# jafarinia/snuffy

Measured on AMD Instinct MI355X. Metric: slides/sec, higher is better.
Workload: dtype f32; 1 GPU; cfgB: MILNet eval forward, 1 bag/step/rank, N=32768 patches D=768 h=6 Lambda=200 (K=200) depth=1 relu mlp x4; parallelism=bag-parallel x1, bags_resident_per_rank=8, launch=hip graph replay, rccl_ranks=0

## Files before the change

### snuffy_amd/csrc/rowops.hip

```cpp
#include <math.h>

#include "common.h"
#include "philox.h"
#include "selector.h"

namespace {

constexpr int WG = 256;
constexpr int WAVES = WG / 64;

template <int VEC>
struct VecT;
template <>
struct VecT<4> {
    using type = float4;
};
template <>
struct VecT<1> {
    using type = float;
};

template <int VEC, int NV>
struct RowRegs {
    float v[NV * VEC];
// ... 27 lines not shown
                *reinterpret_cast<float4*>(row + e) = make_float4(r[i * 4], r[i * 4 + 1], r[i * 4 + 2], r[i * 4 + 3]);
            } else {
                row[e] = r[i];
            }
        }
    }
}

template <int VEC, int NV>
__device__ __forceinline__ void store_row_bf16(unsigned short* __restrict__ row, int d, int lane,
                                               const float (&r)[NV * VEC]) {
#pragma unroll
    for (int i = 0; i < NV; ++i) {
        int e = (i * 64 + lane) * VEC;
        if (e < d) {
            if constexpr (VEC == 4) {
                uint2 p;
                p.x = pack_bf16x2(r[i * 4], r[i * 4 + 1]);
                p.y = pack_bf16x2(r[i * 4 + 2], r[i * 4 + 3]);
                *reinterpret_cast<uint2*>(row + e) = p;
            } else {
                row[e] = f32_to_bf16_bits(r[i]);
            }
        }
    }
}

template <int VEC, int NV, int LN>
__global__ __launch_bounds__(WG) void critic_kernel(const float* __restrict__ x, int64_t n, int d,
                                                    const float* __restrict__ w, const float* __restrict__ b,
                                                    int c_out, float* __restrict__ scores, float eps,
                                                    unsigned short* __restrict__ xhat,
                                                    unsigned int* __restrict__ sel_hist,
                                                    const float* __restrict__ gamma = nullptr,
                                                    const float* __restrict__ beta = nullptr) {
    const int lane = threadIdx.x & 63;
    const int wave = threadIdx.x >> 6;
    const float inv_d = 1.0f / (float)d;
    __shared__ unsigned int s_hist[snf::SEL_BINS];
    if (sel_hist) {
        for (int i = threadIdx.x; i < snf::SEL_BINS; i += WG) s_hist[i] = 0;
        __syncthreads();
    }
    float w0[NV * VEC];
    load_row<VEC, NV>(w, d, lane, w0);
    const float b0 = b ? b[0] : 0.f;
// ... 35 lines not shown
            for (int i = 0; i < NV; ++i) {
#pragma unroll
                for (int t = 0; t < VEC; ++t) {
                    int e = (i * 64 + lane) * VEC + t;
                    float dv = (e < d) ? (r[i * VEC + t] - mean) : 0.f;
                    s2 = fmaf(dv, dv, s2);
                }
            }
            const float var = wave_sum(s2) * inv_d;
            const float rstd = 1.0f / sqrtf(var + eps);
#pragma unroll
            for (int i = 0; i < NV * VEC; ++i) r[i] = (r[i] - mean) * rstd;
            if constexpr (LN == 1) store_row_bf16<VEC, NV>(xhat + row * d, d, lane, r);
            if constexpr (LN == 2 && VEC == 4) {
                if (gamma) {
                    float g[NV * VEC], bt[NV * VEC];
                    load_row<VEC, NV>(gamma, d, lane, g);
                    load_row<VEC, NV>(beta, d, lane, bt);
#pragma unroll
                    for (int i = 0; i < NV * VEC; ++i) {
                        r[i] = fmaf(r[i], g[i], bt[i]);
                    }
                }
                unsigned short* o2 = xhat + row * 2 * d;
#pragma unroll
                for (int i = 0; i < NV; ++i) {
                    const int e = (i * 64 + lane) * 4;
                    if (e < d) {
                        uint2 hi, lo;
                        hi.x = pack_bf16x2(r[i * 4], r[i * 4 + 1]);
                        hi.y = pack_bf16x2(r[i * 4 + 2], r[i * 4 + 3]);
                        lo.x = pack_bf16x2(r[i * 4] - __uint_as_float(hi.x << 16), r[i * 4 + 1] - __uint_as_float(hi.x & 0xffff0000u));
                        lo.y = pack_bf16x2(r[i * 4 + 2] - __uint_as_float(hi.y << 16), r[i * 4 + 3] - __uint_as_float(hi.y & 0xffff0000u));
                        unsigned short* o = o2 + 64 * (e >> 5) + (e & 31);
                        *reinterpret_cast<uint2*>(o) = hi;
                        *reinterpret_cast<uint2*>(o + 32) = lo;
                    }
                }
            }
        }
    }
    if (sel_hist) {
        __syncthreads();
        unsigned int* g = sel_hist + (blockIdx.x & (snf::SEL_REPL - 1)) * snf::SEL_BINS;
        for (int i = threadIdx.x; i < snf::SEL_BINS; i += WG) {
            const unsigned int c = s_hist[i];
            if (c) __hip_atomic_fetch_add(&g[i], c, __ATOMIC_RELAXED, __HIP_MEMORY_SCOPE_AGENT);
        }
    }
}

__global__ __launch_bounds__(1024) void colmax_kernel(const float* __restrict__ scores, int64_t n, int c_out,
                                                      float* __restrict__ out_val, int64_t* __restrict__ out_idx) {
    const int c = blockIdx.x;
    float best = -INFINITY;
    int64_t bi = INT64_MAX;
    bool has_nan = false;
    int64_t nan_i = INT64_MAX;
    for (int64_t i = threadIdx.x; i < n; i += blockDim.x) {
        float v = scores[i * c_out + c];
        if (v != v) {
// ... 81 lines not shown
        }
        const float var = wave_sum(s2) * inv_d;
        const float rstd = 1.0f / sqrtf(var + eps);
#pragma unroll
        for (int i = 0; i < NV * VEC; ++i) {
            float v = (r[i] - mean) * rstd;
            if (gamma) v *= g[i];
            if (beta) v += bt[i];
            r[i] = v;
        }
        const int64_t orow = out_row_idx ? out_row_idx[row] : row;
        if (out_f32) store_row_f32<VEC, NV>(out_f32 + orow * d, d, lane, r);
        if (out_bf16 && !split3) store_row_bf16<VEC, NV>(out_bf16 + orow * d, d, lane, r);
        if (out_bf16 && split3 == 1) {
            float lo[NV * VEC];
#pragma unroll
            for (int i = 0; i < NV * VEC; ++i) lo[i] = r[i] - bf16_bits_to_f32(f32_to_bf16_bits(r[i]));
            unsigned short* o3 = out_bf16 + orow * 3 * d;
            store_row_bf16<VEC, NV>(o3, d, lane, r);
            store_row_bf16<VEC, NV>(o3 + d, d, lane, r);
            store_row_bf16<VEC, NV>(o3 + 2 * d, d, lane, lo);
        }
        if constexpr (VEC == 4) {
            if (out_bf16 && split3 == 2) {
                unsigned short* o2 = out_bf16 + orow * 2 * d;
#pragma unroll
                for (int i = 0; i < NV; ++i) {
                    const int e = (i * 64 + lane) * 4;
                    if (e < d) {
                        uint2 hi, lo;
                        hi.x = pack_bf16x2(r[i * 4], r[i * 4 + 1]);
                        hi.y = pack_bf16x2(r[i * 4 + 2], r[i * 4 + 3]);
                        lo.x = pack_bf16x2(r[i * 4] - __uint_as_float(hi.x << 16), r[i * 4 + 1] - __uint_as_float(hi.x & 0xffff0000u));
                        lo.y = pack_bf16x2(r[i * 4 + 2] - __uint_as_float(hi.y << 16), r[i * 4 + 3] - __uint_as_float(hi.y & 0xffff0000u));
                        unsigned short* o = o2 + 64 * (e >> 5) + (e & 31);
                        *reinterpret_cast<uint2*>(o) = hi;
                        *reinterpret_cast<uint2*>(o + 32) = lo;
                    }
                }
            }
        }
        if (lane == 0) {
            if (mean_out) mean_out[orow] = mean;
            if (rstd_out) rstd_out[orow] = rstd;
        }
    }
}

template <int VEC, int NV>
__device__ __forceinline__ void load_row_bf16(const unsigned short* __restrict__ row, int d, int lane, float (&r)[NV * VEC]) {
#pragma unroll
    for (int i = 0; i < NV; ++i) {
        int e = (i * 64 + lane) * VEC;
        if constexpr (VEC == 4) {
            uint2 t = make_uint2(0u, 0u);
            if (e < d) t = *reinterpret_cast<const uint2*>(row + e);
            r[i * 4 + 0] = __uint_as_float(t.x << 16);
            r[i * 4 + 1] = __uint_as_float(t.x & 0xffff0000u);
            r[i * 4 + 2] = __uint_as_float(t.y << 16);
            r[i * 4 + 3] = __uint_as_float(t.y & 0xffff0000u);
        } else {
            r[i] = (e < d) ? bf16_bits_to_f32(row[e]) : 0.f;
        }
// ... 721 lines not shown
    for (int i = 0; i < NV; ++i) {
        int e = (i * 64 + lane) * VEC;
        if (e < d) {
            if constexpr (VEC == 4) {
                uint2 p = *reinterpret_cast<const uint2*>(row + e);
                r[i * 4 + 0] += __uint_as_float(p.x << 16);
                r[i * 4 + 1] += __uint_as_float(p.x & 0xffff0000u);
                r[i * 4 + 2] += __uint_as_float(p.y << 16);
                r[i * 4 + 3] += __uint_as_float(p.y & 0xffff0000u);
            } else {
                r[i] += bf16_bits_to_f32(row[e]);
            }
        }
    }
}

template <int VEC, int NV, bool DEFER = false>
__global__ __launch_bounds__(WG) void ln_colsum_kernel(const float* __restrict__ z, int64_t n, int d, float eps,
                                                       const unsigned short* __restrict__ add_bf16,
                                                       const float* __restrict__ add_bias,
                                                       const int32_t* __restrict__ slot_map,
                                                       const float* __restrict__ delta_rows,
                                                       float* __restrict__ z_out,
                                                       float* __restrict__ partial ,
                                                       const int* __restrict__ vl = nullptr, int vl_bags = 0,
                                                       const float* __restrict__ slabs = nullptr,
                                                       const int32_t* __restrict__ tile_map = nullptr, int tiles_n = 0) {
    const int lane = threadIdx.x & 63;
    const int wave = threadIdx.x >> 6;
    int bid = blockIdx.x, gdim = gridDim.x;
    if (vl) {
        const int* __restrict__ dsc = vl + 4 * vl[4 * vl_bags + bid];
        const int64_t row0 = dsc[1];
        bid -= dsc[0];
        n = dsc[2];
        gdim = dsc[3];
        z += row0 * d;
        if (add_bf16) add_bf16 += row0 * d;
        if (slot_map) slot_map += row0;
        if (z_out) z_out += row0 * d;
    }
    float acc[NV * VEC];
#pragma unroll
    for (int i = 0; i < NV * VEC; ++i) acc[i] = 0.f;
    float bias_r[NV * VEC];
    if (add_bias) load_row<VEC, NV>(add_bias, d, lane, bias_r);
    const float inv_d = 1.0f / (float)d;
    const int64_t rstride = (int64_t)gdim * WAVES;
    float nz[NV * VEC];
    uint2 nb[NV];
    constexpr int NCB = DEFER ? (NV * VEC * 64 + 255) / 256 : 1;
    float ns[DEFER ? NV * VEC : 1];
    int mp_n[NCB], mp_nn[NCB];
    auto lookup = [&](int64_t row, int (&mp)[NCB]) __attribute__((always_inline)) {
        const int trow = __builtin_amdgcn_readfirstlane((int)(row >> 8));
#pragma unroll
        for (int cb = 0; cb < NCB; ++cb) mp[cb] = cb < tiles_n ? tile_map[(int64_t)trow * tiles_n + cb] : 0;
    };
    auto issue = [&](int64_t row) __attribute__((always_inline)) {
        load_row<VEC, NV>(z + row * d, d, lane, nz);
        if constexpr (DEFER) {
#pragma unroll
            for (int i = 0; i < NV; ++i) {
                const int sl = mp_n[i * 64 * VEC / 256];
#pragma unroll
                for (int t = 0; t < VEC; ++t) ns[i * VEC + t] = 0.f;
                if (sl) {
                    const int e = (i * 64 + lane) * VEC;
                    const float* __restrict__ sp = slabs + ((int64_t)(sl - 1) * 256 + (row & 255)) * 256 + (e & 255);
                    if constexpr (VEC == 4) {
                        if (e < d) {
                            const float4 t4 = *reinterpret_cast<const float4*>(sp);
                            ns[i * 4 + 0] = t4.x, ns[i * 4 + 1] = t4.y, ns[i * 4 + 2] = t4.z, ns[i * 4 + 3] = t4.w;
                        }
                    } else {
                        if (e < d) ns[i] = *sp;
                    }
                }
            }
        }
        if constexpr (VEC == 4) {
            if (add_bf16) {
#pragma unroll
                for (int i = 0; i < NV; ++i) {
                    const int e = (i * 64 + lane) * 4;
                    nb[i] = (e < d) ? *reinterpret_cast<const uint2*>(add_bf16 + row * d + e) : make_uint2(0u, 0u);
                }
            }
        }
    };
    int64_t row = (int64_t)bid * WAVES + wave;
    if constexpr (DEFER) {
        if (row < n) lookup(row, mp_n);
    }
    if (row < n) issue(row);
    if constexpr (DEFER) {
        if (row + rstride < n) lookup(row + rstride, mp_nn);
    }
    for (; row < n; row += rstride) {
        float r[NV * VEC];
#pragma unroll
        for (int i = 0; i < NV * VEC; ++i) r[i] = nz[i];
        if constexpr (DEFER) {
#pragma unroll
            for (int i = 0; i < NV; ++i) {
                if (mp_n[i * 64 * VEC / 256]) {
#pragma unroll
                    for (int t = 0; t < VEC; ++t) r[i * VEC + t] += ns[i * VEC + t];
                }
            }
#pragma unroll
            for (int cb = 0; cb < NCB; ++cb) mp_n[cb] = mp_nn[cb];
        }
        if constexpr (VEC == 4) {
            if (add_bf16) {
#pragma unroll
                for (int i = 0; i < NV; ++i) {
                    r[i * 4 + 0] += __uint_as_float(nb[i].x << 16);
                    r[i * 4 + 1] += __uint_as_float(nb[i].x & 0xffff0000u);
                    r[i * 4 + 2] += __uint_as_float(nb[i].y << 16);
                    r[i * 4 + 3] += __uint_as_float(nb[i].y & 0xffff0000u);
                }
            }
        } else {
            if (add_bf16) add_row_bf16<VEC, NV>(add_bf16 + row * d, d, lane, r);
        }
        if (row + rstride < n) issue(row + rstride);
        if constexpr (DEFER) {
            if (row + 2 * rstride < n) lookup(row + 2 * rstride, mp_nn);
        }
        if (add_bias) {
#pragma unroll
            for (int i = 0; i < NV * VEC; ++i) r[i] += bias_r[i];
        }
        if (slot_map) {
            int sl = slot_map[row];
            if (sl >= 0) {
                float dr[NV * VEC];
                load_row<VEC, NV>(delta_rows + (int64_t)sl * d, d, lane, dr);
#pragma unroll
                for (int i = 0; i < NV * VEC; ++i) r[i] += dr[i];
            }
        }
        if (z_out) store_row_f32<VEC, NV>(z_out + row * d, d, lane, r);
        float s1 = 0.f;
#pragma unroll
        for (int i = 0; i < NV * VEC; ++i) s1 += r[i];
        const float mean = wave_sum(s1) * inv_d;
        float s2 = 0.f;
#pragma unroll
        for (int i = 0; i < NV; ++i) {
#pragma unroll
            for (int t = 0; t < VEC; ++t) {
                int e = (i * 64 + lane) * VEC + t;
                float dv = (e < d) ? (r[i * VEC + t] - mean) : 0.f;
                s2 = fmaf(dv, dv, s2);
            }
        }
        const float rstd = 1.0f / sqrtf(wave_sum(s2) * inv_d + eps);
#pragma unroll
        for (int i = 0; i < NV * VEC; ++i) acc[i] += (r[i] - mean) * rstd;
    }
    extern __shared__ float lds[];
    float* mine = lds + wave * (NV * VEC * 64);
#pragma unroll
    for (int i = 0; i < NV * VEC; ++i) mine[i * 64 + lane] = acc[i];
    __syncthreads();
    if (wave == 0) {
#pragma unroll
        for (int i = 0; i < NV; ++i) {
#pragma unroll
            for (int t = 0; t < VEC; ++t) {
                float s = 0.f;
                for (int w2 = 0; w2 < WAVES; ++w2) s += lds[w2 * (NV * VEC * 64) + (i * VEC + t) * 64 + lane];
                int e = (i * 64 + lane) * VEC + t;
                if (e < d) partial[(int64_t)blockIdx.x * d + e] = s;
            }
        }
    }
}

constexpr int HEAD_NSLICE = 16;
__global__ __launch_bounds__(256) void ln_colreduce_kernel(const float* __restrict__ partial, int nparts, int d,
                                                           float* __restrict__ partial2 ,
                                                           const int* __restrict__ vl = nullptr) {
    __shared__ float red[4][64];
    if (vl) {
        const int* __restrict__ dsc = vl + 4 * blockIdx.z;
        partial += (int64_t)dsc[0] * d;
        nparts = dsc[3];
        partial2 += (int64_t)blockIdx.z * HEAD_NSLICE * d;
    }
    const int c = threadIdx.x & 63, wv = threadIdx.x >> 6;
    const int e = blockIdx.x * 64 + c;
    const int sl = blockIdx.y;
    float s = 0.f;
    if (e < d)
        for (int p = sl + HEAD_NSLICE * wv; p < nparts; p += HEAD_NSLICE * 4) s += partial[(int64_t)p * d + e];
    red[wv][c] = s;
    __syncthreads();
    if (wv == 0 && e < d) partial2[(int64_t)sl * d + e] = ((red[0][c] + red[1][c]) + red[2][c]) + red[3][c];
// ... 42 lines not shown
        const int opts[] = {1, 2, 3, 4, 6, 8};
        for (int o : opts)
            if (o >= need) {
                *cfg = {4, o};
                return true;
            }
        return false;
    }
    int need = (d + 63) / 64;
    const int opts[] = {1, 2, 3, 4, 8, 16, 32};
    for (int o : opts)
        if (o >= need) {
            *cfg = {1, o};
            return true;
        }
    return false;
}

inline int row_grid(int64_t n) {
    int64_t want = (n + WAVES - 1) / WAVES;
    int64_t cap = (int64_t)snf::cu_count() * 8;
    return (int)(want < cap ? (want > 0 ? want : 1) : cap);
}

#define SNF_ROW_DISPATCH(cfg, ...)                                \
    do {                                                          \
        if (cfg.vec == 4) {                                       \
            switch (cfg.nv) {                                     \
                case 1: { constexpr int VEC = 4, NV = 1; __VA_ARGS__; } break; \
                case 2: { constexpr int VEC = 4, NV = 2; __VA_ARGS__; } break; \
                case 3: { constexpr int VEC = 4, NV = 3; __VA_ARGS__; } break; \
                case 4: { constexpr int VEC = 4, NV = 4; __VA_ARGS__; } break; \
                case 6: { constexpr int VEC = 4, NV = 6; __VA_ARGS__; } break; \
                default: { constexpr int VEC = 4, NV = 8; __VA_ARGS__; } break; \
            }                                                     \
        } else {                                                  \
            switch (cfg.nv) {                                     \
                case 1: { constexpr int VEC = 1, NV = 1; __VA_ARGS__; } break; \
                case 2: { constexpr int VEC = 1, NV = 2; __VA_ARGS__; } break; \
                case 3: { constexpr int VEC = 1, NV = 3; __VA_ARGS__; } break; \
                case 4: { constexpr int VEC = 1, NV = 4; __VA_ARGS__; } break; \
                case 8: { constexpr int VEC = 1, NV = 8; __VA_ARGS__; } break; \
                case 16: { constexpr int VEC = 1, NV = 16; __VA_ARGS__; } break; \
                default: { constexpr int VEC = 1, NV = 32; __VA_ARGS__; } break; \
            }                                                     \
        }                                                         \
// ... 84 lines not shown
}

__global__ __launch_bounds__(256) void mil_loss_bwd_kernel(const float* __restrict__ grad_out, const float* __restrict__ fwd, const int64_t* __restrict__ argmax,
                                                           int64_t n, int c, float* __restrict__ d_ins, float* __restrict__ small) {
    const float go = grad_out[0];
    const int64_t total = n * c;
    for (int64_t i = (int64_t)blockIdx.x * 256 + threadIdx.x; i < total; i += (int64_t)gridDim.x * 256) {
        const int64_t row = i / c;
        const int j = (int)(i - row * c);
        d_ins[i] = row == argmax[j] ? go * fwd[2 + 2 * c + j] : 0.f;
    }
    if (blockIdx.x == 0 && threadIdx.x <= c) small[threadIdx.x] = go * (threadIdx.x < c ? fwd[2 + c + threadIdx.x] : fwd[1]);
}

extern "C" {

int snf_critic_f32(const float* x, int64_t n, int d, const float* w, const float* b, int c_out, float* scores,
                   float* colmax_val, int64_t* colmax_idx, snf_stream_t stream) {
    SNF_REQUIRE(x && w && scores, "snf_critic_f32: null pointer");
    SNF_REQUIRE(n >= 1 && d >= 1 && c_out >= 1, "snf_critic_f32: bad shape n=%lld d=%d c=%d", (long long)n, d, c_out);
    RowCfg cfg;
    SNF_REQUIRE(pick_row_cfg(d, aligned16(x) && aligned16(w), &cfg), "snf_critic_f32: d=%d too wide (max 2048)", d);
    hipStream_t s = snf::as_stream(stream);
    SNF_ROW_DISPATCH(cfg, hipLaunchKernelGGL((critic_kernel<VEC, NV, 0>), dim3(row_grid(n)), dim3(WG), 0, s, x, n, d, w,
                                              b, c_out, scores, 0.f, (unsigned short*)nullptr, (unsigned int*)nullptr));
    int rc = snf::check_launch("critic_kernel");
    if (rc) return rc;
    if (colmax_val || colmax_idx) {
        hipLaunchKernelGGL(colmax_kernel, dim3(c_out), dim3(1024), 0, s, scores, n, c_out, colmax_val, colmax_idx);
        rc = snf::check_launch("colmax_kernel");
    }
    return rc;
}

int snf_critic_ln_f32(const float* x, int64_t n, int d, const float* w, const float* b, int c_out, float* scores,
                      float eps, void* xhat_bf16, snf_stream_t stream) {
    SNF_REQUIRE(x && w && scores && xhat_bf16, "snf_critic_ln_f32: null pointer");
    SNF_REQUIRE(n >= 1 && d >= 1 && c_out >= 1, "snf_critic_ln_f32: bad shape n=%lld d=%d c=%d", (long long)n, d, c_out);
    RowCfg cfg;
    SNF_REQUIRE(pick_row_cfg(d, aligned16(x) && aligned16(w) && aligned16(xhat_bf16), &cfg),
                "snf_critic_ln_f32: d=%d too wide (max 2048)", d);
    hipStream_t s = snf::as_stream(stream);
    SNF_ROW_DISPATCH(cfg, hipLaunchKernelGGL((critic_kernel<VEC, NV, 1>), dim3(row_grid(n)), dim3(WG), 0, s, x, n, d, w,
                                              b, c_out, scores, eps, reinterpret_cast<unsigned short*>(xhat_bf16),
                                              (unsigned int*)nullptr));
    return snf::check_launch("critic_kernel<ln>");
}

int snf_critic_select_f32(const float* x, int64_t n, int d, const float* w, const float* b, float* scores, float eps,
                          void* xhat_bf16, void* selector_state, snf_stream_t stream) {
    SNF_REQUIRE(x && w && scores && selector_state, "snf_critic_select_f32: null pointer");
    SNF_REQUIRE(n >= 1 && d >= 1, "snf_critic_select_f32: bad shape n=%lld d=%d", (long long)n, d);
    SNF_REQUIRE(aligned16(selector_state), "snf_critic_select_f32: state must be 16-byte aligned");
    RowCfg cfg;
    SNF_REQUIRE(pick_row_cfg(d, aligned16(x) && aligned16(w) && (!xhat_bf16 || aligned16(xhat_bf16)), &cfg),
                "snf_critic_select_f32: d=%d too wide (max 2048)", d);
    hipStream_t s = snf::as_stream(stream);
    unsigned int* hist = reinterpret_cast<snf::SelectorState*>(selector_state)->hist;
    if (xhat_bf16) {
        SNF_ROW_DISPATCH(cfg, hipLaunchKernelGGL((critic_kernel<VEC, NV, 1>), dim3(row_grid(n)), dim3(WG), 0, s, x, n, d, w, b,
                                                  1, scores, eps, reinterpret_cast<unsigned short*>(xhat_bf16), hist));
    } else {
        SNF_ROW_DISPATCH(cfg, hipLaunchKernelGGL((critic_kernel<VEC, NV, 0>), dim3(row_grid(n)), dim3(WG), 0, s, x, n, d, w,
                                                  b, 1, scores, 0.f, (unsigned short*)nullptr, hist));
    }
    return snf::check_launch("critic_kernel<select>");
}

int snf_critic_ln_hl_f32(const float* x, int64_t n, int d, const float* w, const float* b, int c_out, float* scores,
                         const float* gamma, const float* beta, float eps, void* out_hl, void* selector_state,
                         snf_stream_t stream) {
    SNF_REQUIRE(x && w && scores && out_hl && (!gamma == !beta), "snf_critic_ln_hl_f32: null pointer (gamma and beta: both or neither)");
    SNF_REQUIRE(n >= 1 && d >= 32 && d % 32 == 0 && c_out >= 1, "snf_critic_ln_hl_f32: bad shape n=%lld d=%d c=%d (d % 32 == 0)",
                (long long)n, d, c_out);
    SNF_REQUIRE(!selector_state || (c_out == 1 && aligned16(selector_state)), "snf_critic_ln_hl_f32: the selector needs one class "
                "and a 16-byte aligned state");
    SNF_REQUIRE(aligned16(x) && aligned16(w) && (!gamma || (aligned16(gamma) && aligned16(beta))) && aligned16(out_hl),
                "snf_critic_ln_hl_f32: buffers must be 16-byte aligned");
    RowCfg cfg;
    SNF_REQUIRE(pick_row_cfg(d, true, &cfg) && cfg.vec == 4, "snf_critic_ln_hl_f32: d=%d too wide (max 2048)", d);
    hipStream_t s = snf::as_stream(stream);
    unsigned int* hist = selector_state ? reinterpret_cast<snf::SelectorState*>(selector_state)->hist : nullptr;
    switch (cfg.nv) {
#define SNF_CRITIC_HL_CASE(N)                                                                                              \
    case N:                                                                                                                 \
        hipLaunchKernelGGL((critic_kernel<4, N, 2>), dim3(row_grid(n)), dim3(WG), 0, s, x, n, d, w, b, c_out, scores, eps,  \
                           reinterpret_cast<unsigned short*>(out_hl), hist, gamma, beta);                                   \
        break;
        SNF_CRITIC_HL_CASE(1)
        SNF_CRITIC_HL_CASE(2)
        SNF_CRITIC_HL_CASE(3)
        SNF_CRITIC_HL_CASE(4)
        SNF_CRITIC_HL_CASE(6)
        default:
            SNF_CRITIC_HL_CASE(8)
#undef SNF_CRITIC_HL_CASE
    }
    return snf::check_launch("critic_kernel<ln, hl>");
}

int snf_layernorm_rows_f32(const float* x, int64_t n, int d, const int32_t* slot_map, const float* patch_rows,
                           const float* gamma, const float* beta, float eps, float* out_f32, void* out_bf16,
                           float* mean, float* rstd, const int64_t* out_row_idx, snf_stream_t stream) {
    SNF_REQUIRE(x, "snf_layernorm_rows_f32: null x");
    SNF_REQUIRE(n >= 1 && d >= 1, "snf_layernorm_rows_f32: bad shape");
    SNF_REQUIRE(!slot_map || patch_rows, "snf_layernorm_rows_f32: slot_map without patch_rows");
    bool al = aligned16(x) && (!patch_rows || aligned16(patch_rows)) && (!gamma || aligned16(gamma)) &&
              (!beta || aligned16(beta)) && (!out_f32 || aligned16(out_f32)) && (!out_bf16 || aligned16(out_bf16));
    RowCfg cfg;
    SNF_REQUIRE(pick_row_cfg(d, al, &cfg), "snf_layernorm_rows_f32: d=%d too wide (max 2048)", d);
    hipStream_t s = snf::as_stream(stream);
    SNF_ROW_DISPATCH(cfg, hipLaunchKernelGGL((layernorm_rows_kernel<VEC, NV>), dim3(row_grid(n)), dim3(WG), 0, s, x, n, d,
                                              slot_map, patch_rows, gamma, beta, eps, out_f32,
                                              reinterpret_cast<unsigned short*>(out_bf16), mean, rstd, out_row_idx, 0));
    return snf::check_launch("layernorm_rows_kernel");
}

int snf_layernorm_rows_split3_f32(const float* x, int64_t n, int d, const int32_t* slot_map, const float* patch_rows,
                                  const float* gamma, const float* beta, float eps, void* out_bf16, snf_stream_t stream) {
    SNF_REQUIRE(x && out_bf16, "snf_layernorm_rows_split3_f32: null pointer");
    SNF_REQUIRE(n >= 1 && d >= 1, "snf_layernorm_rows_split3_f32: bad shape");
    SNF_REQUIRE(!slot_map || patch_rows, "snf_layernorm_rows_split3_f32: slot_map without patch_rows");
    bool al = aligned16(x) && (!patch_rows || aligned16(patch_rows)) && (!gamma || aligned16(gamma)) &&
              (!beta || aligned16(beta)) && aligned16(out_bf16);
    RowCfg cfg;
    SNF_REQUIRE(pick_row_cfg(d, al, &cfg), "snf_layernorm_rows_split3_f32: d=%d too wide (max 2048)", d);
    hipStream_t s = snf::as_stream(stream);
    SNF_ROW_DISPATCH(cfg, hipLaunchKernelGGL((layernorm_rows_kernel<VEC, NV>), dim3(row_grid(n)), dim3(WG), 0, s, x, n, d,
                                              slot_map, patch_rows, gamma, beta, eps, (float*)nullptr,
                                              reinterpret_cast<unsigned short*>(out_bf16), (float*)nullptr, (float*)nullptr,
                                              (const int64_t*)nullptr, 1));
    return snf::check_launch("layernorm_rows_kernel<split3>");
}

int snf_layernorm_bwd_blocks(int64_t n) { return row_grid(n); }

int snf_layernorm_rows_bwd_f32(const float* x, int64_t n, int d, const void* dy, int dy_dtype, int64_t dy_stride,
                               const float* gamma, float eps, const float* residual, float* dx, void* dx_bf16,
                               float* partials, snf_stream_t stream) {
    SNF_REQUIRE(x && dy, "snf_layernorm_rows_bwd_f32: null pointer");
    SNF_REQUIRE(n >= 1 && d >= 1, "snf_layernorm_rows_bwd_f32: bad shape");
    SNF_REQUIRE(dy_dtype == SNF_DT_F32 || dy_dtype == SNF_DT_BF16, "snf_layernorm_rows_bwd_f32: bad dy dtype %d", dy_dtype);
    SNF_REQUIRE(dy_stride == 0 || dy_stride >= d, "snf_layernorm_rows_bwd_f32: bad dy row pitch");
    bool al = aligned16(x) && aligned16(dy) && (!gamma || aligned16(gamma)) && (!residual || aligned16(residual)) &&
              (!dx || aligned16(dx)) && (!dx_bf16 || aligned16(dx_bf16)) && dy_stride % 4 == 0;
    RowCfg cfg;
    SNF_REQUIRE(pick_row_cfg(d, al, &cfg), "snf_layernorm_rows_bwd_f32: d=%d too wide (max 2048)", d);
    hipStream_t s = snf::as_stream(stream);
    SNF_ROW_DISPATCH(cfg, hipLaunchKernelGGL((ln_bwd_rows_kernel<VEC, NV>), dim3(row_grid(n)), dim3(WG), 0, s, x, n, d, dy,
                                              dy_dtype == SNF_DT_BF16 ? 1 : 0, dy_stride, gamma, eps, residual, dx,
                                              reinterpret_cast<unsigned short*>(dx_bf16), partials));
// ... 109 lines not shown
            default: SNF_COLSUM_DROP(true, 4); break;
        }
    } else {
        switch (nch) {
            case 1: SNF_COLSUM_DROP(false, 1); break;
            case 2: SNF_COLSUM_DROP(false, 2); break;
            default: SNF_COLSUM_DROP(false, 4); break;
        }
    }
#undef SNF_COLSUM_DROP
    return snf::check_launch("colsum_fused_dropout_kernel");
}

int snf_layernorm_rows_hl_f32(const float* x, int64_t n, int d, const int32_t* slot_map, const float* patch_rows,
                              const float* gamma, const float* beta, float eps, void* out_bf16, snf_stream_t stream) {
    SNF_REQUIRE(x && out_bf16, "snf_layernorm_rows_hl_f32: null pointer");
    SNF_REQUIRE(n >= 1 && d >= 32 && d % 32 == 0, "snf_layernorm_rows_hl_f32: d=%d must be a multiple of 32", d);
    SNF_REQUIRE(!slot_map || patch_rows, "snf_layernorm_rows_hl_f32: slot_map without patch_rows");
    SNF_REQUIRE(aligned16(x) && (!patch_rows || aligned16(patch_rows)) && (!gamma || aligned16(gamma)) && (!beta || aligned16(beta)) &&
                    aligned16(out_bf16), "snf_layernorm_rows_hl_f32: buffers must be 16-byte aligned");
    RowCfg cfg;
    SNF_REQUIRE(pick_row_cfg(d, true, &cfg) && cfg.vec == 4, "snf_layernorm_rows_hl_f32: d=%d too wide (max 2048)", d);
    hipStream_t s = snf::as_stream(stream);
    SNF_ROW_DISPATCH(cfg, hipLaunchKernelGGL((layernorm_rows_kernel<VEC, NV>), dim3(row_grid(n)), dim3(WG), 0, s, x, n, d,
                                              slot_map, patch_rows, gamma, beta, eps, (float*)nullptr,
                                              reinterpret_cast<unsigned short*>(out_bf16), (float*)nullptr, (float*)nullptr,
                                              (const int64_t*)nullptr, 2));
    return snf::check_launch("layernorm_rows_kernel<hl>");
}

int snf_layernorm_rows_hl_patch_f32(const float* x, const float* addend, int64_t n, int d, const int64_t* out_row_idx,
                                    const float* gamma, const float* beta, float eps, void* out_hl, snf_stream_t stream) {
    SNF_REQUIRE(x && out_hl && out_row_idx, "snf_layernorm_rows_hl_patch_f32: null pointer");
    SNF_REQUIRE(n >= 1 && d >= 32 && d % 32 == 0, "snf_layernorm_rows_hl_patch_f32: d=%d must be a multiple of 32", d);
    SNF_REQUIRE(aligned16(x) && (!addend || aligned16(addend)) && (!gamma || aligned16(gamma)) && (!beta || aligned16(beta)) &&
                    aligned16(out_hl), "snf_layernorm_rows_hl_patch_f32: buffers must be 16-byte aligned");
    RowCfg cfg;
    SNF_REQUIRE(pick_row_cfg(d, true, &cfg) && cfg.vec == 4, "snf_layernorm_rows_hl_patch_f32: d=%d too wide (max 2048)", d);
    hipStream_t s = snf::as_stream(stream);
    SNF_ROW_DISPATCH(cfg, hipLaunchKernelGGL((layernorm_rows_kernel<VEC, NV>), dim3(row_grid(n)), dim3(WG), 0, s, x, n, d,
                                              (const int32_t*)nullptr, (const float*)nullptr, gamma, beta, eps, (float*)nullptr,
                                              reinterpret_cast<unsigned short*>(out_hl), (float*)nullptr, (float*)nullptr,
                                              out_row_idx, 2, addend));
    return snf::check_launch("layernorm_rows_kernel<hl patch>");
}

int snf_split_hl_f32(const float* x, int64_t ldx, int64_t m, int k, void* out_bf16, snf_stream_t stream) {
    SNF_REQUIRE(x && out_bf16, "snf_split_hl_f32: null pointer");
    SNF_REQUIRE(m >= 1 && k >= 32 && k % 32 == 0 && ldx >= k && ldx % 4 == 0, "snf_split_hl_f32: bad shape m=%lld k=%d ldx=%lld",
                (long long)m, k, (long long)ldx);
    SNF_REQUIRE(aligned16(x) && aligned16(out_bf16), "snf_split_hl_f32: buffers must be 16-byte aligned");
    const int64_t total = m * (k >> 3);
    int64_t blocks = (total + 255) / 256;
    const int64_t cap = (int64_t)snf::cu_count() * 16;
    if (blocks > cap) blocks = cap;
    hipLaunchKernelGGL(split_hl_kernel, dim3((int)blocks), dim3(256), 0, snf::as_stream(stream), x, ldx, m, k,
                       reinterpret_cast<unsigned short*>(out_bf16));
    return snf::check_launch("split_hl_kernel");
}

int snf_split3_f32(const float* x, int64_t ldx, int64_t m, int k, void* out_bf16, snf_stream_t stream) {
    SNF_REQUIRE(x && out_bf16, "snf_split3_f32: null pointer");
    SNF_REQUIRE(m >= 1 && k >= 8 && k % 8 == 0 && ldx >= k && ldx % 4 == 0, "snf_split3_f32: bad shape m=%lld k=%d ldx=%lld",
// ... 226 lines not shown

static int ln_mean_head_impl(const float* z, int64_t n, int d, const float* slabs, const int32_t* tile_map, int tiles_n,
                             const void* add_bf16, const float* add_bias, const int32_t* slot_map, const float* delta_rows,
                             float* z_out, const float* gamma, const float* beta, float eps, const float* w_head,
                             const float* b_head, int c_out, float* logits, float* pooled, void* workspace, size_t workspace_bytes,
                             snf_stream_t stream) {
    SNF_REQUIRE(z && w_head && logits && workspace, "snf_ln_mean_head_f32: null pointer");
    SNF_REQUIRE(!slot_map || delta_rows, "snf_ln_mean_head_f32: slot_map without delta_rows");
    SNF_REQUIRE(n >= 1 && d >= 1 && c_out >= 1, "snf_ln_mean_head_f32: bad shape");
    const int parts = ln_head_parts(n);
    if (workspace_bytes < ((size_t)parts + HEAD_NSLICE) * d * sizeof(float)) {
        snf::set_error("snf_ln_mean_head_f32: workspace %zu < %zu", workspace_bytes,
                       ((size_t)parts + HEAD_NSLICE) * d * sizeof(float));
        return SNF_EWORKSPACE;
    }
    RowCfg cfg;
    const bool al = aligned16(z) && (!add_bf16 || aligned16(add_bf16)) && (!add_bias || aligned16(add_bias)) &&
                    (!delta_rows || aligned16(delta_rows)) && (!z_out || aligned16(z_out));
    SNF_REQUIRE(pick_row_cfg(d, al, &cfg), "snf_ln_mean_head_f32: d=%d too wide (max 2048)", d);
    hipStream_t s = snf::as_stream(stream);
    float* partial = reinterpret_cast<float*>(workspace);
    float* partial2 = partial + (size_t)parts * d;
    if (tile_map) {
        SNF_ROW_DISPATCH(cfg, hipLaunchKernelGGL((ln_colsum_kernel<VEC, NV, true>), dim3(parts), dim3(WG),
                                                  WAVES * NV * VEC * 64 * sizeof(float), s, z, n, d, eps,
                                                  reinterpret_cast<const unsigned short*>(add_bf16), add_bias, slot_map,
                                                  delta_rows, z_out, partial, nullptr, 0, slabs, tile_map, tiles_n));
    } else {
        SNF_ROW_DISPATCH(cfg, hipLaunchKernelGGL((ln_colsum_kernel<VEC, NV>), dim3(parts), dim3(WG),
                                                  WAVES * NV * VEC * 64 * sizeof(float), s, z, n, d, eps,
                                                  reinterpret_cast<const unsigned short*>(add_bf16), add_bias, slot_map,
                                                  delta_rows, z_out, partial));
    }
    int rc = snf::check_launch("ln_colsum_kernel");
    if (rc) return rc;
    hipLaunchKernelGGL(ln_colreduce_kernel, dim3((d + 63) / 64, HEAD_NSLICE), dim3(256), 0, s, partial, parts, d, partial2);
    rc = snf::check_launch("ln_colreduce_kernel");
    if (rc) return rc;
    hipLaunchKernelGGL(head_gemv_kernel, dim3(c_out), dim3(256), 0, s, partial2, n, d, gamma, beta, w_head, b_head, pooled,
                       logits);
    return snf::check_launch("head_gemv_kernel");
}

int snf_ln_mean_head_f32(const float* z, int64_t n, int d, const void* add_bf16, const float* add_bias,
                         const int32_t* slot_map, const float* delta_rows, float* z_out, const float* gamma,
                         const float* beta, float eps, const float* w_head, const float* b_head, int c_out, float* logits,
                         float* pooled, void* workspace, size_t workspace_bytes, snf_stream_t stream) {
    return ln_mean_head_impl(z, n, d, nullptr, nullptr, 0, add_bf16, add_bias, slot_map, delta_rows, z_out, gamma, beta, eps, w_head,
                             b_head, c_out, logits, pooled, workspace, workspace_bytes, stream);
}

int snf_ln_mean_head_deferred_f32(const float* z, int64_t n, int d, const float* slabs, const int32_t* tile_map, int tiles_n,
                                  const void* add_bf16, const float* add_bias, const int32_t* slot_map, const float* delta_rows,
                                  float* z_out, const float* gamma, const float* beta, float eps, const float* w_head,
                                  const float* b_head, int c_out, float* logits, float* pooled, void* workspace,
// ... 39 lines not shown
                                int c_out, float* logits, float* pooled, const int32_t* table_dev, void* workspace,
                                size_t workspace_bytes, snf_stream_t stream) {
    SNF_REQUIRE(z && offsets && w_head && logits && workspace && table_dev, "snf_ln_mean_head_varlen_f32: null pointer");
    SNF_REQUIRE(!slot_map || delta_rows, "snf_ln_mean_head_varlen_f32: slot_map without delta_rows");
    SNF_REQUIRE(bags >= 1 && d >= 1 && c_out >= 1, "snf_ln_mean_head_varlen_f32: bad shape");
    int64_t total = 0;
    for (int b = 0; b < bags; ++b) {
        SNF_REQUIRE(offsets[b + 1] > offsets[b], "snf_ln_mean_head_varlen_f32: empty bag %d", b);
        total += ln_head_parts(offsets[b + 1] - offsets[b]);
    }
    const size_t need = ((size_t)total + (size_t)bags * HEAD_NSLICE) * d * sizeof(float);
    if (workspace_bytes < need) {
        snf::set_error("snf_ln_mean_head_varlen_f32: workspace %zu < %zu", workspace_bytes, need);
        return SNF_EWORKSPACE;
    }
    RowCfg cfg;
    const bool al = aligned16(z) && (!add_bf16 || aligned16(add_bf16)) && (!add_bias || aligned16(add_bias)) &&
                    (!delta_rows || aligned16(delta_rows)) && (!z_out || aligned16(z_out));
    SNF_REQUIRE(pick_row_cfg(d, al, &cfg), "snf_ln_mean_head_varlen_f32: d=%d too wide (max 2048)", d);
    hipStream_t s = snf::as_stream(stream);
    float* partial = reinterpret_cast<float*>(workspace);
    float* partial2 = partial + (size_t)total * d;
    const int64_t n_all = offsets[bags];
    SNF_ROW_DISPATCH(cfg, hipLaunchKernelGGL((ln_colsum_kernel<VEC, NV>), dim3((unsigned)total), dim3(WG),
                                              WAVES * NV * VEC * 64 * sizeof(float), s, z, n_all, d, eps,
                                              reinterpret_cast<const unsigned short*>(add_bf16), add_bias, slot_map,
                                              delta_rows, z_out, partial, table_dev, bags));
    int rc = snf::check_launch("ln_colsum_kernel");
    if (rc) return rc;
    hipLaunchKernelGGL(ln_colreduce_kernel, dim3((d + 63) / 64, HEAD_NSLICE, bags), dim3(256), 0, s, partial, 0, d, partial2,
                       table_dev);
    rc = snf::check_launch("ln_colreduce_kernel");
    if (rc) return rc;
    hipLaunchKernelGGL(head_gemv_kernel, dim3(c_out, bags), dim3(256), 0, s, partial2, n_all, d, gamma, beta, w_head, b_head,
                       pooled, logits, table_dev);
    return snf::check_launch("head_gemv_kernel");
}

int snf_dropout_mask_f32(float dropout_p, uint64_t seed, uint64_t offset, int h, int64_t n, int k, float* mask,
                         snf_stream_t stream) {
    SNF_REQUIRE(mask && h >= 1 && n >= 1 && k >= 1, "snf_dropout_mask_f32: bad arguments");
    SNF_REQUIRE(dropout_p >= 0.f && dropout_p < 1.f, "snf_dropout_mask_f32: dropout_p=%f outside [0, 1)", dropout_p);
    const snf::DropoutState st = snf::make_dropout(dropout_p, seed, offset);
    const int64_t groups = (int64_t)h * n * ((k + 3) >> 2);
    hipLaunchKernelGGL(dropout_mask_kernel, dim3((unsigned)((groups + 255) / 256)), dim3(256), 0, snf::as_stream(stream), st, h, n, k,
                       mask, groups);
    return snf::check_launch("dropout_mask_kernel");
}

int snf_mil_loss_f32(const float* ins, int64_t n, int c, const float* logits, const float* label, const float* w, const float* pos_weight,
// ... 19 lines not shown
```

Baseline: 905.7 slides/s.

## Cap row-kernel grids at resident occupancy and coalesce hi/lo bf16 stores

Row kernels (critic, layernorm, ln_colsum) now launch a grid capped at occupancy-resident blocks when there are enough rows, so persistent blocks loop over logical blocks. ln_colsum is restructured to iterate logical blocks with a prefetch cursor that carries across block boundaries, keeping the per-logical-block partial layout. Separately, the hi/lo split bf16 store swaps halves between lane pairs via DPP so each lane writes one 16-byte store instead of two 8-byte ones. The aim is lower block scheduling overhead and wider stores. The cost is extra control flow, an occupancy query cached per kernel, and a per-logical-block syncthreads.

```diff
diff --git a/snuffy_amd/csrc/rowops.hip b/snuffy_amd/csrc/rowops.hip
--- a/snuffy_amd/csrc/rowops.hip
+++ b/snuffy_amd/csrc/rowops.hip
@@ -1,4 +1,6 @@
 #include <math.h>
+
+#include <unordered_map>
 
 #include "common.h"
 #include "philox.h"
@@ -73,6 +75,28 @@
             } else {
                 row[e] = f32_to_bf16_bits(r[i]);
             }
+        }
+    }
+}
+
+template <int NV>
+__device__ __forceinline__ void store_row_hl(unsigned short* __restrict__ o2, int d, int lane, const float (&r)[NV * 4]) {
+    const bool odd = lane & 1;
+#pragma unroll
+    for (int i = 0; i < NV; ++i) {
+        const int e = (i * 64 + lane) * 4;
+        uint2 hi, lo;
+        hi.x = pack_bf16x2(r[i * 4], r[i * 4 + 1]);
+        hi.y = pack_bf16x2(r[i * 4 + 2], r[i * 4 + 3]);
+        lo.x = pack_bf16x2(r[i * 4] - __uint_as_float(hi.x << 16), r[i * 4 + 1] - __uint_as_float(hi.x & 0xffff0000u));
+        lo.y = pack_bf16x2(r[i * 4 + 2] - __uint_as_float(hi.y << 16), r[i * 4 + 3] - __uint_as_float(hi.y & 0xffff0000u));
+        const uint2 give = odd ? hi : lo;
+        uint2 got;
+        got.x = (unsigned int)__builtin_amdgcn_update_dpp(0, (int)give.x, 0xb1, 0xf, 0xf, false);
+        got.y = (unsigned int)__builtin_amdgcn_update_dpp(0, (int)give.y, 0xb1, 0xf, 0xf, false);
+        if (e < d) {
+            unsigned short* o = o2 + 64 * (e >> 5) + (e & 31) + (odd ? 28 : 0);
+            *reinterpret_cast<uint4*>(o) = odd ? make_uint4(got.x, got.y, lo.x, lo.y) : make_uint4(hi.x, hi.y, got.x, got.y);
         }
     }
 }
@@ -154,21 +178,7 @@
                         r[i] = fmaf(r[i], g[i], bt[i]);
                     }
                 }
-                unsigned short* o2 = xhat + row * 2 * d;
-#pragma unroll
-                for (int i = 0; i < NV; ++i) {
-                    const int e = (i * 64 + lane) * 4;
-                    if (e < d) {
-                        uint2 hi, lo;
-                        hi.x = pack_bf16x2(r[i * 4], r[i * 4 + 1]);
-                        hi.y = pack_bf16x2(r[i * 4 + 2], r[i * 4 + 3]);
-                        lo.x = pack_bf16x2(r[i * 4] - __uint_as_float(hi.x << 16), r[i * 4 + 1] - __uint_as_float(hi.x & 0xffff0000u));
-                        lo.y = pack_bf16x2(r[i * 4 + 2] - __uint_as_float(hi.y << 16), r[i * 4 + 3] - __uint_as_float(hi.y & 0xffff0000u));
-                        unsigned short* o = o2 + 64 * (e >> 5) + (e & 31);
-                        *reinterpret_cast<uint2*>(o) = hi;
-                        *reinterpret_cast<uint2*>(o + 32) = lo;
-                    }
-                }
+                store_row_hl<NV>(xhat + row * 2 * d, d, lane, r);
             }
         }
     }
@@ -296,23 +306,7 @@
             store_row_bf16<VEC, NV>(o3 + 2 * d, d, lane, lo);
         }
         if constexpr (VEC == 4) {
-            if (out_bf16 && split3 == 2) {
-                unsigned short* o2 = out_bf16 + orow * 2 * d;
-#pragma unroll
-                for (int i = 0; i < NV; ++i) {
-                    const int e = (i * 64 + lane) * 4;
-                    if (e < d) {
-                        uint2 hi, lo;
-                        hi.x = pack_bf16x2(r[i * 4], r[i * 4 + 1]);
-                        hi.y = pack_bf16x2(r[i * 4 + 2], r[i * 4 + 3]);
-                        lo.x = pack_bf16x2(r[i * 4] - __uint_as_float(hi.x << 16), r[i * 4 + 1] - __uint_as_float(hi.x & 0xffff0000u));
-                        lo.y = pack_bf16x2(r[i * 4 + 2] - __uint_as_float(hi.y << 16), r[i * 4 + 3] - __uint_as_float(hi.y & 0xffff0000u));
-                        unsigned short* o = o2 + 64 * (e >> 5) + (e & 31);
-                        *reinterpret_cast<uint2*>(o) = hi;
-                        *reinterpret_cast<uint2*>(o + 32) = lo;
-                    }
-                }
-            }
+            if (out_bf16 && split3 == 2) store_row_hl<NV>(out_bf16 + orow * 2 * d, d, lane, r);
         }
         if (lane == 0) {
             if (mean_out) mean_out[orow] = mean;
@@ -1080,31 +1074,38 @@
                                                        const int32_t* __restrict__ slot_map,
                                                        const float* __restrict__ delta_rows,
                                                        float* __restrict__ z_out,
-                                                       float* __restrict__ partial ,
+                                                       float* __restrict__ partial , int lgrid,
                                                        const int* __restrict__ vl = nullptr, int vl_bags = 0,
                                                        const float* __restrict__ slabs = nullptr,
                                                        const int32_t* __restrict__ tile_map = nullptr, int tiles_n = 0) {
     const int lane = threadIdx.x & 63;
-    const int wave = threadIdx.x >> 6;
-    int bid = blockIdx.x, gdim = gridDim.x;
-    if (vl) {
-        const int* __restrict__ dsc = vl + 4 * vl[4 * vl_bags + bid];
-        const int64_t row0 = dsc[1];
-        bid -= dsc[0];
-        n = dsc[2];
-        gdim = dsc[3];
-        z += row0 * d;
-        if (add_bf16) add_bf16 += row0 * d;
-        if (slot_map) slot_map += row0;
-        if (z_out) z_out += row0 * d;
-    }
+    const int wave = __builtin_amdgcn_readfirstlane(threadIdx.x >> 6);
+    struct Pos {
+        int lb;
+        int64_t row, n, rstride, row0;
+    };
+    auto enter = [&](Pos& p) __attribute__((always_inline)) {
+        int bid = p.lb;
+        if (vl) {
+            const int* __restrict__ dsc = vl + 4 * vl[4 * vl_bags + p.lb];
+            bid -= dsc[0];
+            p.row0 = dsc[1];
+            p.n = dsc[2];
+            p.rstride = (int64_t)dsc[3] * WAVES;
+        }
+        p.row = (int64_t)bid * WAVES + wave;
+    };
+    auto seek = [&](Pos& p) __attribute__((always_inline)) {
+        while (p.row >= p.n) {
+            p.lb += (int)gridDim.x;
+            if (p.lb >= lgrid) break;
+            enter(p);
+        }
+    };
     float acc[NV * VEC];
-#pragma unroll
-    for (int i = 0; i < NV * VEC; ++i) acc[i] = 0.f;
     float bias_r[NV * VEC];
     if (add_bias) load_row<VEC, NV>(add_bias, d, lane, bias_r);
     const float inv_d = 1.0f / (float)d;
-    const int64_t rstride = (int64_t)gdim * WAVES;
     float nz[NV * VEC];
     uint2 nb[NV];
     constexpr int NCB = DEFER ? (NV * VEC * 64 + 255) / 256 : 1;
@@ -1147,94 +1148,110 @@
             }
         }
     };
-    int64_t row = (int64_t)bid * WAVES + wave;
+    Pos p1 = {(int)blockIdx.x, 0, n, (int64_t)lgrid * WAVES, 0};
+    enter(p1);
+    seek(p1);
+    Pos p2 = p1;
+    if (p1.lb < lgrid) {
+        if constexpr (DEFER) lookup(p1.row0 + p1.row, mp_n);
+        issue(p1.row0 + p1.row);
+        p2.row += p2.rstride;
+        seek(p2);
+    }
     if constexpr (DEFER) {
-        if (row < n) lookup(row, mp_n);
-    }
-    if (row < n) issue(row);
-    if constexpr (DEFER) {
-        if (row + rstride < n) lookup(row + rstride, mp_nn);
-    }
-    for (; row < n; row += rstride) {
-        float r[NV * VEC];
-#pragma unroll
-        for (int i = 0; i < NV * VEC; ++i) r[i] = nz[i];
-        if constexpr (DEFER) {
+        if (p2.lb < lgrid) lookup(p2.row0 + p2.row, mp_nn);
+    }
+    extern __shared__ float lds[];
+    for (int lb = blockIdx.x; lb < lgrid; lb += (int)gridDim.x) {
+#pragma unroll
+        for (int i = 0; i < NV * VEC; ++i) acc[i] = 0.f;
+        while (p1.lb == lb) {
+            const int64_t row = p1.row0 + p1.row;
+            float r[NV * VEC];
+#pragma unroll
+            for (int i = 0; i < NV * VEC; ++i) r[i] = nz[i];
+            if constexpr (DEFER) {
+#pragma unroll
+                for (int i = 0; i < NV; ++i) {
+                    if (mp_n[i * 64 * VEC / 256]) {
+#pragma unroll
+                        for (int t = 0; t < VEC; ++t) r[i * VEC + t] += ns[i * VEC + t];
+                    }
+                }
+#pragma unroll
+                for (int cb = 0; cb < NCB; ++cb) mp_n[cb] = mp_nn[cb];
+            }
+            if constexpr (VEC == 4) {
+                if (add_bf16) {
+#pragma unroll
+                    for (int i = 0; i < NV; ++i) {
+                        r[i * 4 + 0] += __uint_as_float(nb[i].x << 16);
+                        r[i * 4 + 1] += __uint_as_float(nb[i].x & 0xffff0000u);
+                        r[i * 4 + 2] += __uint_as_float(nb[i].y << 16);
+                        r[i * 4 + 3] += __uint_as_float(nb[i].y & 0xffff0000u);
+                    }
+                }
+            } else {
+                if (add_bf16) add_row_bf16<VEC, NV>(add_bf16 + row * d, d, lane, r);
+            }
+            p1 = p2;
+            if (p1.lb < lgrid) {
+                issue(p1.row0 + p1.row);
+                p2.row += p2.rstride;
+                seek(p2);
+            }
+            if constexpr (DEFER) {
+                if (p2.lb < lgrid) lookup(p2.row0 + p2.row, mp_nn);
+            }
+            if (add_bias) {
+#pragma unroll
+                for (int i = 0; i < NV * VEC; ++i) r[i] += bias_r[i];
+            }
+            if (slot_map) {
+                int sl = slot_map[row];
+                if (sl >= 0) {
+                    float dr[NV * VEC];
+                    load_row<VEC, NV>(delta_rows + (int64_t)sl * d, d, lane, dr);
+#pragma unroll
+                    for (int i = 0; i < NV * VEC; ++i) r[i] += dr[i];
+                }
+            }
+            if (z_out) store_row_f32<VEC, NV>(z_out + row * d, d, lane, r);
+            float s1 = 0.f;
+#pragma unroll
+            for (int i = 0; i < NV * VEC; ++i) s1 += r[i];
+            const float mean = wave_sum(s1) * inv_d;
+            float s2 = 0.f;
 #pragma unroll
             for (int i = 0; i < NV; ++i) {
-                if (mp_n[i * 64 * VEC / 256]) {
-#pragma unroll
-                    for (int t = 0; t < VEC; ++t) r[i * VEC + t] += ns[i * VEC + t];
+#pragma unroll
+                for (int t = 0; t < VEC; ++t) {
+                    int e = (i * 64 + lane) * VEC + t;
+                    float dv = (e < d) ? (r[i * VEC + t] - mean) : 0.f;
+                    s2 = fmaf(dv, dv, s2);
                 }
             }
-#pragma unroll
-            for (int cb = 0; cb < NCB; ++cb) mp_n[cb] = mp_nn[cb];
-        }
-        if constexpr (VEC == 4) {
-            if (add_bf16) {
-#pragma unroll
-                for (int i = 0; i < NV; ++i) {
-                    r[i * 4 + 0] += __uint_as_float(nb[i].x << 16);
-                    r[i * 4 + 1] += __uint_as_float(nb[i].x & 0xffff0000u);
-                    r[i * 4 + 2] += __uint_as_float(nb[i].y << 16);
-                    r[i * 4 + 3] += __uint_as_float(nb[i].y & 0xffff0000u);
+            const float rstd = 1.0f / sqrtf(wave_sum(s2) * inv_d + eps);
+#pragma unroll
+            for (int i = 0; i < NV * VEC; ++i) acc[i] += (r[i] - mean) * rstd;
+        }
+        float* mine = lds + wave * (NV * VEC * 64);
+#pragma unroll
+        for (int i = 0; i < NV * VEC; ++i) mine[i * 64 + lane] = acc[i];
+        __syncthreads();
+        if (wave == 0) {
+#pragma unroll
+            for (int i = 0; i < NV; ++i) {
+#pragma unroll
+                for (int t = 0; t < VEC; ++t) {
+                    float s = 0.f;
+                    for (int w2 = 0; w2 < WAVES; ++w2) s += lds[w2 * (NV * VEC * 64) + (i * VEC + t) * 64 + lane];
+                    int e = (i * 64 + lane) * VEC + t;
+                    if (e < d) partial[(int64_t)lb * d + e] = s;
                 }
             }
-        } else {
-            if (add_bf16) add_row_bf16<VEC, NV>(add_bf16 + row * d, d, lane, r);
-        }
-        if (row + rstride < n) issue(row + rstride);
-        if constexpr (DEFER) {
-            if (row + 2 * rstride < n) lookup(row + 2 * rstride, mp_nn);
-        }
-        if (add_bias) {
-#pragma unroll
-            for (int i = 0; i < NV * VEC; ++i) r[i] += bias_r[i];
-        }
-        if (slot_map) {
-            int sl = slot_map[row];
-            if (sl >= 0) {
-                float dr[NV * VEC];
-                load_row<VEC, NV>(delta_rows + (int64_t)sl * d, d, lane, dr);
-#pragma unroll
-                for (int i = 0; i < NV * VEC; ++i) r[i] += dr[i];
-            }
-        }
-        if (z_out) store_row_f32<VEC, NV>(z_out + row * d, d, lane, r);
-        float s1 = 0.f;
-#pragma unroll
-        for (int i = 0; i < NV * VEC; ++i) s1 += r[i];
-        const float mean = wave_sum(s1) * inv_d;
-        float s2 = 0.f;
-#pragma unroll
-        for (int i = 0; i < NV; ++i) {
-#pragma unroll
-            for (int t = 0; t < VEC; ++t) {
-                int e = (i * 64 + lane) * VEC + t;
-                float dv = (e < d) ? (r[i * VEC + t] - mean) : 0.f;
-                s2 = fmaf(dv, dv, s2);
-            }
-        }
-        const float rstd = 1.0f / sqrtf(wave_sum(s2) * inv_d + eps);
-#pragma unroll
-        for (int i = 0; i < NV * VEC; ++i) acc[i] += (r[i] - mean) * rstd;
-    }
-    extern __shared__ float lds[];
-    float* mine = lds + wave * (NV * VEC * 64);
-#pragma unroll
-    for (int i = 0; i < NV * VEC; ++i) mine[i * 64 + lane] = acc[i];
-    __syncthreads();
-    if (wave == 0) {
-#pragma unroll
-        for (int i = 0; i < NV; ++i) {
-#pragma unroll
-            for (int t = 0; t < VEC; ++t) {
-                float s = 0.f;
-                for (int w2 = 0; w2 < WAVES; ++w2) s += lds[w2 * (NV * VEC * 64) + (i * VEC + t) * 64 + lane];
-                int e = (i * 64 + lane) * VEC + t;
-                if (e < d) partial[(int64_t)blockIdx.x * d + e] = s;
-            }
-        }
+        }
+        if (lb + (int)gridDim.x < lgrid) __syncthreads();
     }
 }
 
@@ -1323,6 +1340,26 @@
     int64_t cap = (int64_t)snf::cu_count() * 8;
     return (int)(want < cap ? (want > 0 ? want : 1) : cap);
 }
+
+constexpr int ROW_TRIPS_MIN = 4;
+template <typename K>
+inline int resident_grid(K kernel, size_t lds_bytes, int logical, int64_t rows) {
+    static thread_local std::unordered_map<const void*, int> per_cu;
+    const void* key = reinterpret_cast<const void*>(kernel);
+    auto it = per_cu.find(key);
+    if (it == per_cu.end()) {
+        int nb = 0;
+        if (hipOccupancyMaxActiveBlocksPerMultiprocessor(&nb, kernel, WG, lds_bytes) != hipSuccess) {
+            (void)hipGetLastError();
+            nb = 0;
+        }
+        it = per_cu.emplace(key, nb).first;
+    }
+    const int64_t resident = (int64_t)it->second * snf::cu_count();
+    return resident >= 1 && resident < logical && rows >= resident * WAVES * ROW_TRIPS_MIN ? (int)resident : logical;
+}
+#define SNF_ROW_LAUNCH(kernel, logical, rows, lds, stream, ...) \
+    hipLaunchKernelGGL((kernel), dim3(resident_grid((kernel), (lds), (logical), (rows))), dim3(WG), (lds), (stream), __VA_ARGS__)
 
 #define SNF_ROW_DISPATCH(cfg, ...)                                \
     do {                                                          \
@@ -1453,7 +1490,7 @@
     RowCfg cfg;
     SNF_REQUIRE(pick_row_cfg(d, aligned16(x) && aligned16(w), &cfg), "snf_critic_f32: d=%d too wide (max 2048)", d);
     hipStream_t s = snf::as_stream(stream);
-    SNF_ROW_DISPATCH(cfg, hipLaunchKernelGGL((critic_kernel<VEC, NV, 0>), dim3(row_grid(n)), dim3(WG), 0, s, x, n, d, w,
+    SNF_ROW_DISPATCH(cfg, SNF_ROW_LAUNCH((critic_kernel<VEC, NV, 0>), row_grid(n), n, 0, s, x, n, d, w,
                                               b, c_out, scores, 0.f, (unsigned short*)nullptr, (unsigned int*)nullptr));
     int rc = snf::check_launch("critic_kernel");
     if (rc) return rc;
@@ -1472,7 +1509,7 @@
     SNF_REQUIRE(pick_row_cfg(d, aligned16(x) && aligned16(w) && aligned16(xhat_bf16), &cfg),
                 "snf_critic_ln_f32: d=%d too wide (max 2048)", d);
     hipStream_t s = snf::as_stream(stream);
-    SNF_ROW_DISPATCH(cfg, hipLaunchKernelGGL((critic_kernel<VEC, NV, 1>), dim3(row_grid(n)), dim3(WG), 0, s, x, n, d, w,
+    SNF_ROW_DISPATCH(cfg, SNF_ROW_LAUNCH((critic_kernel<VEC, NV, 1>), row_grid(n), n, 0, s, x, n, d, w,
                                               b, c_out, scores, eps, reinterpret_cast<unsigned short*>(xhat_bf16),
                                               (unsigned int*)nullptr));
     return snf::check_launch("critic_kernel<ln>");
@@ -1489,10 +1526,10 @@
     hipStream_t s = snf::as_stream(stream);
     unsigned int* hist = reinterpret_cast<snf::SelectorState*>(selector_state)->hist;
     if (xhat_bf16) {
-        SNF_ROW_DISPATCH(cfg, hipLaunchKernelGGL((critic_kernel<VEC, NV, 1>), dim3(row_grid(n)), dim3(WG), 0, s, x, n, d, w, b,
+        SNF_ROW_DISPATCH(cfg, SNF_ROW_LAUNCH((critic_kernel<VEC, NV, 1>), row_grid(n), n, 0, s, x, n, d, w, b,
                                                   1, scores, eps, reinterpret_cast<unsigned short*>(xhat_bf16), hist));
     } else {
-        SNF_ROW_DISPATCH(cfg, hipLaunchKernelGGL((critic_kernel<VEC, NV, 0>), dim3(row_grid(n)), dim3(WG), 0, s, x, n, d, w,
+        SNF_ROW_DISPATCH(cfg, SNF_ROW_LAUNCH((critic_kernel<VEC, NV, 0>), row_grid(n), n, 0, s, x, n, d, w,
                                                   b, 1, scores, 0.f, (unsigned short*)nullptr, hist));
     }
     return snf::check_launch("critic_kernel<select>");
@@ -1515,7 +1552,7 @@
     switch (cfg.nv) {
 #define SNF_CRITIC_HL_CASE(N)                                                                                              \
     case N:                                                                                                                 \
-        hipLaunchKernelGGL((critic_kernel<4, N, 2>), dim3(row_grid(n)), dim3(WG), 0, s, x, n, d, w, b, c_out, scores, eps,  \
+        SNF_ROW_LAUNCH((critic_kernel<4, N, 2>), row_grid(n), n, 0, s, x, n, d, w, b, c_out, scores, eps,  \
                            reinterpret_cast<unsigned short*>(out_hl), hist, gamma, beta);                                   \
         break;
         SNF_CRITIC_HL_CASE(1)
@@ -1541,7 +1578,7 @@
     RowCfg cfg;
     SNF_REQUIRE(pick_row_cfg(d, al, &cfg), "snf_layernorm_rows_f32: d=%d too wide (max 2048)", d);
     hipStream_t s = snf::as_stream(stream);
-    SNF_ROW_DISPATCH(cfg, hipLaunchKernelGGL((layernorm_rows_kernel<VEC, NV>), dim3(row_grid(n)), dim3(WG), 0, s, x, n, d,
+    SNF_ROW_DISPATCH(cfg, SNF_ROW_LAUNCH((layernorm_rows_kernel<VEC, NV>), row_grid(n), n, 0, s, x, n, d,
                                               slot_map, patch_rows, gamma, beta, eps, out_f32,
                                               reinterpret_cast<unsigned short*>(out_bf16), mean, rstd, out_row_idx, 0));
     return snf::check_launch("layernorm_rows_kernel");
@@ -1557,7 +1594,7 @@
     RowCfg cfg;
     SNF_REQUIRE(pick_row_cfg(d, al, &cfg), "snf_layernorm_rows_split3_f32: d=%d too wide (max 2048)", d);
     hipStream_t s = snf::as_stream(stream);
-    SNF_ROW_DISPATCH(cfg, hipLaunchKernelGGL((layernorm_rows_kernel<VEC, NV>), dim3(row_grid(n)), dim3(WG), 0, s, x, n, d,
+    SNF_ROW_DISPATCH(cfg, SNF_ROW_LAUNCH((layernorm_rows_kernel<VEC, NV>), row_grid(n), n, 0, s, x, n, d,
                                               slot_map, patch_rows, gamma, beta, eps, (float*)nullptr,
                                               reinterpret_cast<unsigned short*>(out_bf16), (float*)nullptr, (float*)nullptr,
                                               (const int64_t*)nullptr, 1));
@@ -1713,7 +1750,7 @@
     RowCfg cfg;
     SNF_REQUIRE(pick_row_cfg(d, true, &cfg) && cfg.vec == 4, "snf_layernorm_rows_hl_f32: d=%d too wide (max 2048)", d);
     hipStream_t s = snf::as_stream(stream);
-    SNF_ROW_DISPATCH(cfg, hipLaunchKernelGGL((layernorm_rows_kernel<VEC, NV>), dim3(row_grid(n)), dim3(WG), 0, s, x, n, d,
+    SNF_ROW_DISPATCH(cfg, SNF_ROW_LAUNCH((layernorm_rows_kernel<VEC, NV>), row_grid(n), n, 0, s, x, n, d,
                                               slot_map, patch_rows, gamma, beta, eps, (float*)nullptr,
                                               reinterpret_cast<unsigned short*>(out_bf16), (float*)nullptr, (float*)nullptr,
                                               (const int64_t*)nullptr, 2));
@@ -1729,7 +1766,7 @@
     RowCfg cfg;
     SNF_REQUIRE(pick_row_cfg(d, true, &cfg) && cfg.vec == 4, "snf_layernorm_rows_hl_patch_f32: d=%d too wide (max 2048)", d);
     hipStream_t s = snf::as_stream(stream);
-    SNF_ROW_DISPATCH(cfg, hipLaunchKernelGGL((layernorm_rows_kernel<VEC, NV>), dim3(row_grid(n)), dim3(WG), 0, s, x, n, d,
+    SNF_ROW_DISPATCH(cfg, SNF_ROW_LAUNCH((layernorm_rows_kernel<VEC, NV>), row_grid(n), n, 0, s, x, n, d,
                                               (const int32_t*)nullptr, (const float*)nullptr, gamma, beta, eps, (float*)nullptr,
                                               reinterpret_cast<unsigned short*>(out_hl), (float*)nullptr, (float*)nullptr,
                                               out_row_idx, 2, addend));
@@ -2002,15 +2039,13 @@
     float* partial = reinterpret_cast<float*>(workspace);
     float* partial2 = partial + (size_t)parts * d;
     if (tile_map) {
-        SNF_ROW_DISPATCH(cfg, hipLaunchKernelGGL((ln_colsum_kernel<VEC, NV, true>), dim3(parts), dim3(WG),
-                                                  WAVES * NV * VEC * 64 * sizeof(float), s, z, n, d, eps,
-                                                  reinterpret_cast<const unsigned short*>(add_bf16), add_bias, slot_map,
-                                                  delta_rows, z_out, partial, nullptr, 0, slabs, tile_map, tiles_n));
+        SNF_ROW_DISPATCH(cfg, SNF_ROW_LAUNCH((ln_colsum_kernel<VEC, NV, true>), parts, n, WAVES * NV * VEC * 64 * sizeof(float), s, z, n, d,
+                                                 eps, reinterpret_cast<const unsigned short*>(add_bf16), add_bias, slot_map,
+                                                 delta_rows, z_out, partial, parts, nullptr, 0, slabs, tile_map, tiles_n));
     } else {
-        SNF_ROW_DISPATCH(cfg, hipLaunchKernelGGL((ln_colsum_kernel<VEC, NV>), dim3(parts), dim3(WG),
-                                                  WAVES * NV * VEC * 64 * sizeof(float), s, z, n, d, eps,
-                                                  reinterpret_cast<const unsigned short*>(add_bf16), add_bias, slot_map,
-                                                  delta_rows, z_out, partial));
+        SNF_ROW_DISPATCH(cfg, SNF_ROW_LAUNCH((ln_colsum_kernel<VEC, NV>), parts, n, WAVES * NV * VEC * 64 * sizeof(float), s, z, n, d, eps,
+                                                 reinterpret_cast<const unsigned short*>(add_bf16), add_bias, slot_map,
+                                                 delta_rows, z_out, partial, parts));
     }
     int rc = snf::check_launch("ln_colsum_kernel");
     if (rc) return rc;
@@ -2096,10 +2131,9 @@
     float* partial = reinterpret_cast<float*>(workspace);
     float* partial2 = partial + (size_t)total * d;
     const int64_t n_all = offsets[bags];
-    SNF_ROW_DISPATCH(cfg, hipLaunchKernelGGL((ln_colsum_kernel<VEC, NV>), dim3((unsigned)total), dim3(WG),
-                                              WAVES * NV * VEC * 64 * sizeof(float), s, z, n_all, d, eps,
-                                              reinterpret_cast<const unsigned short*>(add_bf16), add_bias, slot_map,
-                                              delta_rows, z_out, partial, table_dev, bags));
+    SNF_ROW_DISPATCH(cfg, SNF_ROW_LAUNCH((ln_colsum_kernel<VEC, NV>), (int)total, n_all, WAVES * NV * VEC * 64 * sizeof(float), s, z, n_all,
+                                             d, eps, reinterpret_cast<const unsigned short*>(add_bf16), add_bias, slot_map,
+                                             delta_rows, z_out, partial, (int)total, table_dev, bags));
     int rc = snf::check_launch("ln_colsum_kernel");
     if (rc) return rc;
     hipLaunchKernelGGL(ln_colreduce_kernel, dim3((d + 63) / 64, HEAD_NSLICE, bags), dim3(256), 0, s, partial, 0, d, partial2,
```

After: 913.2 slides/s, median of 6. Within noise of the previous version (+0.8%).
